# VIPL-Audio-Visual-Speech-Understanding/SBL_For_Multilingual_Lip_Reading

Measured on AMD Instinct MI355X. Metric: lip-clips/sec fwd+bwd (29x88x88), higher is better.
Workload: dtype f32 (exact 3-way bf16 split, 6 bf16 MFMA products per fp32 product, fp32 accumulate); 1 GPU; full SBL 6+6 (Conv3d stem + ResNet-18 + encoder + SBL decoder) fwd+loss+bwd (BASELINE config 3); matmul_precision=bf16x6, per_gpu_batch=32, global_batch=32, clip=29x88x88, parallelism=dp1, dropout=True, bn=train, issue=graph, hipgraph=True, decoder_streams=2, conv_weight_pack=cached (re-packed when weights change), decoder_schedule=teacher-forced runs batched, coin_patterns=8

## Files before the change

include/sbl_hip.h:

```cpp
#ifndef SBL_HIP_H
#define SBL_HIP_H
#include <stdint.h>
#ifdef __cplusplus
extern "C" {
#endif

#define SBL_ERR_INVALID (-22)
#define SBL_ABI_VERSION 1

typedef void* sbl_stream_t;

const char* sbl_last_error(void);
int sbl_abi_version(void);

int sbl_profile_begin(uint64_t* stamps, int capacity);
int sbl_profile_end(void);
int sbl_profile_used(void);
int sbl_profile_last_slot(void);
int sbl_profile_last_kernel(void);
int sbl_profile_last_route(void);

int sbl_set_matmul_precision(int terms);
int sbl_get_matmul_precision(void);
int sbl_set_tuning(int knob, int value);
// ... 52 lines not shown
int sbl_bn_bwd_apply(const float* dy, const float* y, const float* x, const float* mean, const float* invstd,
                     const float* gamma, const double* sums, float* dx, float* dres, float* dgamma, float* dbeta,
                     long rows, int C, int relu, int accumulate, sbl_stream_t stream);

int sbl_conv_weight_pack(const float* w_oihw, float* w_ohwi, float* w_dgrad , int Cout,
                         int Cin, int KH, int KW, double* zero , int nzero, sbl_stream_t stream);
int sbl_conv_wgrad_unpack(const float* dw_ohwi, float* dw_oihw, int Cout, int Cin, int KH, int KW, int accumulate,
                          sbl_stream_t stream);
int sbl_conv2d_fwd(const float* x, const float* w_ohwi, float* y, double* stats, int stats_zeroed, int NIMG, int H, int W, int Cin,
                   int Cout, int KH, int KW, int stride, int pad, void* ws, long ws_bytes, sbl_stream_t stream);
int sbl_conv2d_dgrad(const float* dy, const float* w_dgrad, float* dx, int NIMG, int H, int W, int Cin, int Cout,
                     int KH, int KW, int stride, int pad, void* ws, long ws_bytes, sbl_stream_t stream);
int sbl_conv2d_dgrad_bnstats(const float* dy, const float* w_dgrad, float* dx, int NIMG, int H, int W, int Cin, int Cout,
                             int KH, int KW, int stride, int pad, void* ws, long ws_bytes, const float* act,
                             const float* pre, const float* mean, const float* invstd, double* sums,
                             int sums_zeroed ,
                             sbl_stream_t stream);
int sbl_conv2d_dgrad_fused(const float* dy, const float* w_dgrad, float* dx, int NIMG, int H, int W, int Cin, int Cout,
                           int KH, int KW, int stride, int pad, void* ws, long ws_bytes, const float* addend,
                           const float* act, const float* pre, const float* mean, const float* invstd, const float* pre2,
                           const float* mean2, const float* invstd2, double* sums, int sums_zeroed, sbl_stream_t stream);
int sbl_conv1x1s2_dgrad_compact(const float* dy, const float* w_dgrad, float* dx_compact, int NIMG, int H, int W, int Cin,
                                int Cout, void* ws, long ws_bytes, sbl_stream_t stream);
int sbl_conv2d_wgrad(const float* x, const float* dy, float* dw_ohwi, int NIMG, int H, int W, int Cin, int Cout,
                     int KH, int KW, int stride, int pad, int dw_zeroed, sbl_stream_t stream);
int sbl_avgpool_fwd(const float* x, float* y, int NIMG, int HW, int C, sbl_stream_t stream);
int sbl_avgpool_bwd(const float* dy, float* dx, int NIMG, int HW, int C, sbl_stream_t stream);

int sbl_dropout(const float* x, float* y, long n, float p, const uint64_t* seed, uint64_t offset,
                sbl_stream_t stream);
int sbl_seed_bump(uint64_t* seed, sbl_stream_t stream);

int sbl_add_layernorm_fwd(const float* x, const float* res, const float* gamma, const float* beta, float* y,
                          float* mean, float* rstd, int M, int D, float eps, float drop_p, const uint64_t* seed,
                          uint64_t offset, sbl_stream_t stream);
int sbl_add_layernorm2_fusion_fwd(const float* x0, const float* x1, const float* res0, const float* res1, const float* gamma0,
                                  const float* gamma1, const float* beta0, const float* beta1, float* xn0, float* xn1, float* mean0,
                                  float* mean1, float* rstd0, float* rstd1, int B, const int* seg_L, int nseg, int D, float eps,
                                  float drop_p, const uint64_t* seed, uint64_t offset0, uint64_t offset1, sbl_stream_t stream);
int sbl_add_layernorm2_fwd(const float* x0, const float* x1, const float* res0, const float* res1, const float* gamma0,
                           const float* gamma1, const float* beta0, const float* beta1, float* y0, float* y1, float* mean0,
                           float* mean1, float* rstd0, float* rstd1, int M, int D, float eps, float drop_p,
                           const uint64_t* seed, uint64_t offset0, uint64_t offset1, sbl_stream_t stream);
int sbl_add_layernorm_bwd(const float* dy, const float* x, const float* res, const float* gamma, const float* mean,
                          const float* rstd, float* dz, float* dx_drop, float* dgamma, float* dbeta, int M, int D,
                          float drop_p, const uint64_t* seed, uint64_t offset, sbl_stream_t stream);
// ... 172 lines not shown
```

sbl_for_multilingual_lip_reading_amd/_lib.py:

```python
import ctypes
import os
from ctypes import c_double, c_float, c_int, c_long, c_uint64, c_void_p

_HERE = os.path.dirname(os.path.abspath(__file__))
LIB_PATH = os.path.join(_HERE, "libsbl_hip.so")

P, I, L, F, U64, D = c_void_p, c_int, c_long, c_float, c_uint64, c_double

SIGNATURES = {
    "sbl_gemm_f32": [I, I, I, I, I, P, L, P, L, P, L, P, I, P, L, I, P, P, L, P],
    "sbl_wgrad_seg_f32": [I, P, L, P, L, P, I, I, P, L, P, P],
    "sbl_wgrad_group_f32": [I, I, P, P, P, P, P, P, P, P, P, P, P, L, P],
    "sbl_colsum_f32": [P, L, P, I, I, I, P],
    "sbl_stem_conv_fwd": [P, P, P, P, I, I, I, I, P],
    "sbl_stem_bn_relu_pool_fwd": [P, P, P, P, P, P, P, I, I, I, P],
    "sbl_stem_bwd_reduce": [P, P, P, P, P, P, P, P, I, I, I, P],
    "sbl_stem_wgrad": [P, P, P, P, P, P, P, P, P, P, P, P, I, I, I, I, P],
    "sbl_stem_conv_fwd_u8": [P, P, P, P, P, P, P, P, P, I, I, I, I, I, I, I, P],
    "sbl_stem_wgrad_u8": [P, P, P, P, P, P, P, P, P, P, P, P, P, P, P, P, P, I, I, I, I, I, I, I, P],
    "sbl_bn_finalize": [P, L, P, P, F, F, P, P, I, P, P],
    "sbl_bn_eval_stats": [P, P, F, P, P, I, P],
    "sbl_bn_apply_fwd": [P, P, P, P, P, P, P, L, I, I, P],
    "sbl_bn_apply_fwd_stats": [P, P, P, L, P, P, F, F, P, P, P, P, P, P, L, I, I, P],
    "sbl_bn_bwd_reduce": [P, P, P, P, P, P, L, I, I, P, L, P],
    "sbl_bn_bwd_apply": [P, P, P, P, P, P, P, P, P, P, P, L, I, I, I, P],
    "sbl_conv_weight_pack": [P, P, P, I, I, I, I, P, I, P],
    "sbl_conv_wgrad_unpack": [P, P, I, I, I, I, I, P],
    "sbl_conv2d_fwd": [P, P, P, P, I, I, I, I, I, I, I, I, I, I, P, L, P],
    "sbl_conv2d_dgrad": [P, P, P, I, I, I, I, I, I, I, I, I, P, L, P],
    "sbl_conv2d_dgrad_bnstats": [P, P, P, I, I, I, I, I, I, I, I, I, P, L, P, P, P, P, P, I, P],
    "sbl_conv2d_dgrad_fused": [P, P, P, I, I, I, I, I, I, I, I, I, P, L, P, P, P, P, P, P, P, P, P, I, P],
    "sbl_conv1x1s2_dgrad_compact": [P, P, P, I, I, I, I, I, P, L, P],
    "sbl_conv2d_wgrad": [P, P, P, I, I, I, I, I, I, I, I, I, I, P],
    "sbl_avgpool_fwd": [P, P, I, I, I, P],
    "sbl_avgpool_bwd": [P, P, I, I, I, P],
    "sbl_dropout": [P, P, L, F, P, U64, P],
    "sbl_seed_bump": [P, P],
    "sbl_add_layernorm_fwd": [P, P, P, P, P, P, P, I, I, F, F, P, U64, P],
    "sbl_add_layernorm_bwd": [P, P, P, P, P, P, P, P, P, P, I, I, F, P, U64, P],
    "sbl_add_pe": [P, P, P, I, I, I, P],
    "sbl_rowscale": [P, P, P, L, I, P],
    "sbl_attention_fwd": [P, L, P, L, P, L, P, L, P, I, P, I, I, I, I, F, F, P, U64, P],
    "sbl_attention_bwd": [P, L, P, L, P, L, P, L, P, P, L, P, L, P, L, I, I, I, I, F, F, P, U64, P],
    "sbl_attention_seg_fwd": [P, L, P, L, P, L, P, L, P, I, P, I, I, P, I, I, F, F, P, U64, P],
    "sbl_attention_seg2_fwd": [P, P, L, P, P, L, P, P, L, P, P, L, P, P, I, I, I, P, I, I, F, F, P, U64, U64, P],
    "sbl_attention_seg_grouped_fwd": [P, L, P, L, P, L, P, L, I, I, P, I, I, I, F, F, P, U64, P],
    "sbl_gemm2_f32": [I, I, I, P, P, L, P, P, L, P, P, L, P, P, I, P, L, P],
    "sbl_gemm2_rows_f32": [I, I, I, P, P, L, P, P, L, P, P, L, P, P, I, P, L, P],
    "sbl_add_layernorm2_fwd": [P, P, P, P, P, P, P, P, P, P, P, P, P, P, I, I, F, F, P, U64, U64, P],
    "sbl_add_layernorm2_fusion_fwd": [P, P, P, P, P, P, P, P, P, P, P, P, P, P, I, P, I, I, F, F, P, U64, U64, P],
    "sbl_attention_seg_bwd": [P, L, P, L, P, L, P, L, P, P, L, P, L, P, L, I, I, P, I, I, F, F, P, U64, P],
    "sbl_embed_pe_seg_fwd": [P, L, P, P, P, I, P, I, I, I, P],
    "sbl_embed_pe_drop2_fwd": [P, P, L, P, P, P, P, I, P, I, I, I, F, P, U64, U64, P],
    "sbl_decoder_tail_fwd": [P, P, P, P, P, P, P, P, L, P, P, L, I, I, I, P, I, I, I, P],
    "sbl_embed_seg_bwd": [P, L, P, P, I, P, I, I, I, P],
# ... 84 lines not shown
```

sbl_for_multilingual_lip_reading_amd/csrc/conv.hip:

```cpp
#include "mfma_gemm.h"
#include "conv_patch.h"
#include "conv_patch_wgrad.h"

SblRouting g_sbl_route = {2, 30};
extern "C" int sbl_set_tuning(int knob, int value) {
    SBL_REQUIRE(knob == 5 || knob == 9, "sbl_set_tuning: no knob %d; the two that remain are 5 (patch-resident 3x3 / stride-1 forward / input gradient: 2 on, "
                "0 the per-tap gather kernels) and 9 (smallest map in pixels that takes the patch-resident weight gradient, 0 = never)", knob);
    if (knob == 5) {
        SBL_REQUIRE(value == 0 || value == 2, "sbl_set_tuning: knob 5 takes 2 (patch-resident kernels) or 0 (per-tap gather kernels), not %d", value);
        g_sbl_route.conv_patch = value;
    } else {
        SBL_REQUIRE(value >= 0, "sbl_set_tuning: negative value");
        g_sbl_route.conv_patch_wgrad = value;
    }
    return 0;
}

static int check_conv(const char* who, int NIMG, int H, int W, int Cin, int Cout, int KH, int KW, int stride, int pad) {
    SBL_REQUIRE(NIMG > 0 && H > 0 && W > 0, "%s: bad image dims %d %d %d", who, NIMG, H, W);
    SBL_REQUIRE(Cin % 16 == 0 && Cout % 16 == 0 && Cin >= 16 && Cout >= 16, "%s: Cin=%d Cout=%d must be multiples of 16", who, Cin, Cout);
    SBL_REQUIRE((KH == 3 && KW == 3 && pad == 1) || (KH == 1 && KW == 1 && pad == 0), "%s: only 3x3/pad1 and 1x1/pad0 (got %dx%d pad %d)", who, KH, KW, pad);
    SBL_REQUIRE(stride == 1 || stride == 2, "%s: stride %d", who, stride);
    SBL_REQUIRE(sbl_fits_u32((long)NIMG * H * W * (long)(Cin > Cout ? Cin : Cout)), "%s: tensor spans more than 2 GiB (buffer descriptor range)", who);
    SBL_REQUIRE((long)NIMG * H * W < (1L << 24) && Cin < (1 << 16) && Cout < (1 << 16), "%s: more than 2^24 pixels (24-bit index arithmetic in the gathers)", who);
// ... 112 lines not shown
    if (stats && !stats_zeroed) SBL_HIP(hipMemsetAsync(stats, 0, sizeof(double) * 2 * Cout, s));
    SBL_REQUIRE(!ws || (sbl_aligned16(ws) && ws_bytes >= (long)sizeof(int) * kConvWsCounters), "sbl_conv2d_fwd: workspace unaligned or < 16 KiB");
    if (KH == 3 && stride == 1) {
        bool done;
        const PatchEpi pe{y, stats, nullptr, nullptr, nullptr, nullptr, nullptr, nullptr, nullptr, nullptr};
        if (stats) done = sbl_launch_conv_patch<false, 1>(x, w, pe, NIMG, H, W, Cin, Cout, SBL_KID_CONV_FWD, s);
        else done = sbl_launch_conv_patch<false, 0>(x, w, pe, NIMG, H, W, Cin, Cout, SBL_KID_CONV_FWD, s);
        if (done) {
            SBL_LAUNCH_CHECK("sbl_conv2d_fwd(patch)");
            return 0;
        }
    }
    if (conv_pm_ok(Ho, Wo, KH, stride)) {
        with_fwd_epi(y, N, stats, rows_pm(NIMG, Ho * Wo), [&](const auto& e) { launch_conv_pm<false>(x, w, g, e, M, N, K, Cin, SBL_KID_CONV_FWD, s); });
        SBL_LAUNCH_CHECK("sbl_conv2d_fwd(pm)");
        return 0;
    }
    const ConvTile tile = conv_tile(N, (long)sbl_cdiv(M, 128) * sbl_cdiv(N, 128), (long)sbl_cdiv(M, 128) * sbl_cdiv(N, 64), true, false);
    with_fwd_epi(y, N, stats, kRowsDirect, [&](const auto& e) { launch_conv_gemm<false>(x, w, g, e, tile, M, N, K, SBL_KID_CONV_FWD, ws, ws_bytes, s); });
    SBL_LAUNCH_CHECK("sbl_conv2d_fwd");
    return 0;
}

struct DgradClass { ConvGeom g; int lin[4]; int M, K, ph, pw; };
static int conv2d_dgrad_impl(const float* dy, const float* wt, float* dx, int NIMG, int H, int W, int Cin, int Cout,
                             int KH, int KW, int stride, int pad, void* ws, long ws_bytes, sbl_stream_t stream,
                             const DgradFuse& f, int compact_out) {
    hipStream_t s = (hipStream_t)stream;
    if (int e = check_conv("sbl_conv2d_dgrad", NIMG, H, W, Cin, Cout, KH, KW, stride, pad)) return e;
    SBL_REQUIRE(dy && wt && dx && sbl_aligned16(dy) && sbl_aligned16(wt), "sbl_conv2d_dgrad: null/unaligned pointer");
    const int Ho = out_dim(H, KH, stride, pad), Wo = out_dim(W, KW, stride, pad);
    const bool fused = f.addend || f.sums;
    if (f.sums) {
        SBL_REQUIRE(f.y && f.x && f.mean && f.inv && (!f.x2 || (f.mean2 && f.inv2)), "sbl_conv2d_dgrad_fused: incomplete BatchNorm operands");
        if (!f.sums_zeroed) SBL_HIP(hipMemsetAsync(f.sums, 0, sizeof(double) * (f.x2 ? 4 : 2) * Cin, s));
    }
    SBL_REQUIRE(!f.addend || f.add_class00 == (stride == 2), "sbl_conv2d_dgrad_fused: the compact addend belongs to stride-2 convolutions (and only to them)");
    SBL_REQUIRE(!compact_out || (KH == 1 && stride == 2 && !fused), "sbl_conv2d_dgrad: compact output is the 1x1 / stride-2 case");
    if (stride == 2) {
        const int N = Cin;
        if (KH == 1 && !compact_out) SBL_HIP(hipMemsetAsync(dx, 0, sizeof(float) * (size_t)NIMG * H * W * Cin, s));
        DgradClass cls[4];
        int nc = 0;
        for (int ph = 0; ph < 2; ++ph)
            for (int pw = 0; pw < 2; ++pw) {
                DgradClass c{ConvGeom{NIMG, (H - ph + 1) / 2, (W - pw + 1) / 2, Ho, Wo, Cout, KH, KW, stride, pad, 1, ph, pw, 0, {0, 0, 0, 0}, {0, 0, 0, 0}}, {0, 0, 0, 0}, 0, 0, ph, pw};
                sbl_geom_finish(c.g);
                for (int kh = 0; kh < KH; ++kh)
                    for (int kw = 0; kw < KW; ++kw)
                        if (((ph + pad - kh) & 1) == 0 && ((pw + pad - kw) & 1) == 0) {
                            c.g.tkh[c.g.ntaps] = kh; c.g.tkw[c.g.ntaps] = kw; c.lin[c.g.ntaps] = kh * KW + kw;
                            ++c.g.ntaps;
                        }
                c.M = NIMG * c.g.OH * c.g.OW;
                c.K = c.g.ntaps * Cout;
                if (c.g.ntaps == 0 || c.M == 0) continue;
                int at = nc++;
                while (at > 0 && cls[at - 1].K < c.K) { cls[at] = cls[at - 1]; --at; }
                cls[at] = c;
            }
        if (nc == 0) return 0;
        SplitCtl sc{nullptr, nullptr, nullptr, sbl_next_stamp_slot(SBL_KID_CONV_DGRAD)};
        const int cmap = compact_out ? 0 : 1;
        long t128 = 0, t128x64 = 0;
        for (int i = 0; i < nc; ++i) {
            t128 += (long)sbl_cdiv(cls[i].M, 128) * sbl_cdiv(N, 128);
            t128x64 += (long)sbl_cdiv(cls[i].M, 128) * sbl_cdiv(N, 64);
        }
        const ConvTile tile = conv_tile(N, t128, t128x64, false, f.sums != nullptr);
        int t0[SBL_MAX_CLASSES + 1];
        long tt = 0;
        for (int i = 0; i <= SBL_MAX_CLASSES; ++i) {
            t0[i] = (int)tt;
            if (i < nc) tt += (long)sbl_cdiv(cls[i].M, conv_tile_m(tile)) * sbl_cdiv(N, conv_tile_n(tile));
        }
        SBL_REQUIRE(tt < (1L << 30), "sbl_conv2d_dgrad: too many tiles");
        with_dgrad_epi(dx, N, f, [&](auto make) {
            with_tile(tile, [&](auto bm, auto bn) {
                constexpr int BM = decltype(bm)::value, BN = decltype(bn)::value;
                using AL = ConvGatherKC<BM, true>;
                using BL = DenseKCTaps<BN>;
                using EPI = decltype(make(kRowsDirect, f.addend, 0L));
                ClassSet<AL, BL, EPI> cs;
                cs.nclass = nc;
                cs.tiles_n = sbl_cdiv(N, BN);
                for (int i = 0; i < SBL_MAX_CLASSES; ++i) {
                    const DgradClass& c = cls[i < nc ? i : 0];
                    const float* add = (f.addend && c.ph == 0 && c.pw == 0) ? f.addend : nullptr;
                    cs.al[i] = AL{dy, c.g, c.M};
                    cs.bl[i] = BL{wt, (long)KH * KW * Cout, N, Cout, {c.lin[0], c.lin[1], c.lin[2], c.lin[3]}};
                    cs.epi[i] = make(RowMap{cmap, c.g.OH, c.g.OW, H, W, c.ph, c.pw}, add, (long)N);
                    cs.M[i] = c.M; cs.K[i] = c.K; cs.t0[i] = t0[i];
                }
                cs.t0[SBL_MAX_CLASSES] = t0[SBL_MAX_CLASSES];
                sbl_note_route(5, sbl_route_tile(BM, BN), 0, 0);
                sbl_with_prec([&](auto p) {
                    hipLaunchKernelGGL((sbl_conv_classes_kernel<AL, BL, EPI, BM, BN, decltype(p)::value>), dim3((unsigned)tt), dim3(256), 0, s, cs, sc, N);
                });
            });
        });
        SBL_LAUNCH_CHECK("sbl_conv2d_dgrad(classes)");
        return 0;
    }
    const int M = NIMG * H * W, N = Cin, K = KH * KW * Cout;
    ConvGeom g{NIMG, H, W, Ho, Wo, Cout, KH, KW, stride, pad, 0, 0, 0, 0, {0, 0, 0, 0}, {0, 0, 0, 0}};
    sbl_geom_finish(g);
    SBL_REQUIRE(!ws || (sbl_aligned16(ws) && ws_bytes >= (long)sizeof(int) * kConvWsCounters), "sbl_conv2d_dgrad: workspace unaligned or < 16 KiB");
    if (KH == 3 && stride == 1) {
        bool done;
        const PatchEpi pe{dx, f.sums, f.addend, f.y, f.x, f.mean, f.inv, f.x2, f.mean2, f.inv2};
        if (f.sums) done = sbl_launch_conv_patch<true, 2>(dy, wt, pe, NIMG, H, W, Cout, Cin, SBL_KID_CONV_DGRAD, s);
        else if (f.addend) done = sbl_launch_conv_patch<true, 3>(dy, wt, pe, NIMG, H, W, Cout, Cin, SBL_KID_CONV_DGRAD, s);
        else done = sbl_launch_conv_patch<true, 0>(dy, wt, pe, NIMG, H, W, Cout, Cin, SBL_KID_CONV_DGRAD, s);
// ... 16 lines not shown
    SBL_LAUNCH_CHECK("sbl_conv2d_dgrad");
    return 0;
}
static const DgradFuse kNoFuse{nullptr, 0, nullptr, nullptr, nullptr, nullptr, nullptr, nullptr, nullptr, nullptr};
extern "C" int sbl_conv2d_dgrad(const float* dy, const float* wt, float* dx, int NIMG, int H, int W, int Cin, int Cout,
                                int KH, int KW, int stride, int pad, void* ws, long ws_bytes, sbl_stream_t stream) {
    return conv2d_dgrad_impl(dy, wt, dx, NIMG, H, W, Cin, Cout, KH, KW, stride, pad, ws, ws_bytes, stream, kNoFuse, 0);
}
extern "C" int sbl_conv2d_dgrad_bnstats(const float* dy, const float* wt, float* dx, int NIMG, int H, int W, int Cin, int Cout,
                                        int KH, int KW, int stride, int pad, void* ws, long ws_bytes, const float* act,
                                        const float* pre, const float* mean, const float* invstd, double* sums,
                                        int sums_zeroed, sbl_stream_t stream) {
    SBL_REQUIRE(act && pre && mean && invstd && sums, "sbl_conv2d_dgrad_bnstats: null statistics operand");
    return conv2d_dgrad_impl(dy, wt, dx, NIMG, H, W, Cin, Cout, KH, KW, stride, pad, ws, ws_bytes, stream,
                             DgradFuse{nullptr, 0, act, pre, mean, invstd, nullptr, nullptr, nullptr, sums, sums_zeroed}, 0);
}
extern "C" int sbl_conv2d_dgrad_fused(const float* dy, const float* wt, float* dx, int NIMG, int H, int W, int Cin, int Cout,
                                      int KH, int KW, int stride, int pad, void* ws, long ws_bytes, const float* addend,
                                      const float* act, const float* pre, const float* mean, const float* invstd,
                                      const float* pre2, const float* mean2, const float* invstd2, double* sums,
                                      int sums_zeroed, sbl_stream_t stream) {
    return conv2d_dgrad_impl(dy, wt, dx, NIMG, H, W, Cin, Cout, KH, KW, stride, pad, ws, ws_bytes, stream,
                             DgradFuse{addend, addend && stride == 2, act, pre, mean, invstd, pre2, mean2, invstd2, sums, sums_zeroed}, 0);
}
extern "C" int sbl_conv1x1s2_dgrad_compact(const float* dy, const float* wt, float* dx_compact, int NIMG, int H, int W, int Cin,
                                           int Cout, void* ws, long ws_bytes, sbl_stream_t stream) {
    return conv2d_dgrad_impl(dy, wt, dx_compact, NIMG, H, W, Cin, Cout, 1, 1, 2, 0, ws, ws_bytes, stream, kNoFuse, 1);
}

static inline int wgrad_splits(long target, long tiles, int K) {
    int splits = (int)((target + tiles - 1) / tiles);
    if (splits > K / 256) splits = K / 256;
    return splits < 1 ? 1 : splits;
}
extern "C" int sbl_conv2d_wgrad(const float* x, const float* dy, float* dw, int NIMG, int H, int W, int Cin, int Cout,
                                int KH, int KW, int stride, int pad, int dw_zeroed, sbl_stream_t stream) {
    hipStream_t s = (hipStream_t)stream;
    if (int e = check_conv("sbl_conv2d_wgrad", NIMG, H, W, Cin, Cout, KH, KW, stride, pad)) return e;
    SBL_REQUIRE(x && dy && dw && sbl_aligned16(x) && sbl_aligned16(dy), "sbl_conv2d_wgrad: null/unaligned pointer");
    const int Ho = out_dim(H, KH, stride, pad), Wo = out_dim(W, KW, stride, pad);
    const int M = Cout, N = KH * KW * Cin, K = NIMG * Ho * Wo;
    ConvGeom g{NIMG, Ho, Wo, H, W, Cin, KH, KW, stride, pad, 0, 0, 0, 0, {0, 0, 0, 0}, {0, 0, 0, 0}};
    sbl_geom_finish(g);
    if (!dw_zeroed) SBL_HIP(hipMemsetAsync(dw, 0, sizeof(float) * (size_t)M * N, s));
    const bool big = M >= 128 && N >= 1152 && !(stride == 2 && sbl_wg_s2_small);
    const int wg_target = stride == 2 ? sbl_wg_s2_target : (big ? 1536 : 3072);
// ... 121 lines not shown
```

sbl_for_multilingual_lip_reading_amd/csrc/tile_loaders.h:

```cpp
#pragma once
#include "sbl_common.h"

#define SBL_BK 16
#define SBL_BUF_BYTES 0x80000000u
#define SBL_OOB 0xC0000000u

typedef __amdgpu_buffer_rsrc_t sbl_rsrc;
__device__ __forceinline__ sbl_rsrc sbl_make_rsrc(const float* p) {
    return __builtin_amdgcn_make_buffer_rsrc(const_cast<float*>(p), 0, (int)SBL_BUF_BYTES, 0x00020000);
}
__device__ __forceinline__ float4 sbl_ld4(sbl_rsrc r, unsigned off) {
    const f32x4 v = __builtin_bit_cast(f32x4, __builtin_amdgcn_raw_buffer_load_b128(r, (int)off, 0, 0));
    return make_float4(v[0], v[1], v[2], v[3]);
}
__device__ __forceinline__ float sbl_ld1(sbl_rsrc r, unsigned off) {
    return __builtin_bit_cast(float, __builtin_amdgcn_raw_buffer_load_b32(r, (int)off, 0, 0));
}
static inline bool sbl_fits_u32(long elems) { return elems >= 0 && elems * 4 <= (long)SBL_BUF_BYTES; }

template <int BR, class Regs>
__device__ __forceinline__ void sbl_store_kc(float (*lds)[BR + 4], const Regs& r, int tid) {
    const int kq = (tid & 3) * 4;
#pragma unroll
    for (int ps = 0; ps < BR / 64; ++ps) {
// ... 54 lines not shown
            } else {
                r.v[ps].x = sbl_ld1(s.rs, ok && k + 0 < kend ? o + 0 : SBL_OOB);
                r.v[ps].y = sbl_ld1(s.rs, ok && k + 1 < kend ? o + 4 : SBL_OOB);
                r.v[ps].z = sbl_ld1(s.rs, ok && k + 2 < kend ? o + 8 : SBL_OOB);
                r.v[ps].w = sbl_ld1(s.rs, ok && k + 3 < kend ? o + 12 : SBL_OOB);
            }
        }
    }
    __device__ __forceinline__ void accum(const Regs&, float4&) const {}
    __device__ __forceinline__ int col(const State&) const { return 0; }
    __device__ __forceinline__ void store(float (*lds)[BR + 4], const State&, const Regs& r, int tid) const { sbl_store_kc<BR>(lds, r, tid); }
};

template <int BR>
struct DenseKCTaps {
    static constexpr bool kColSum = false;
    static constexpr bool kKC = true;
    static constexpr bool kDenseOperand = false;
    const float* p;
    long ld;
    int rows;
    int C;
    int lin[4];
    struct State {
        sbl_rsrc rs;
        unsigned ro[BR / 64];
        int kq;
    };
    struct Regs {
        float4 v[BR / 64];
    };
    __device__ __forceinline__ void init(State& s, int r0, int tid) const {
        s.rs = sbl_make_rsrc(p);
        s.kq = (tid & 3) * 4;
#pragma unroll
        for (int ps = 0; ps < BR / 64; ++ps) {
            const int r = r0 + ps * 64 + (tid >> 2);
            s.ro[ps] = r < rows ? (unsigned)(((long)r * ld + s.kq) * 4) : SBL_OOB;
        }
    }
    __device__ __forceinline__ void load(const State& s, int k0, int kend, Regs& r) const {
        const int t = k0 / C;
        int l = lin[0];
#pragma unroll
        for (int u = 1; u < 4; ++u)
            if (u == t) l = lin[u];
        const unsigned kb = (unsigned)(l * C + (k0 - t * C)) * 4;
#pragma unroll
        for (int ps = 0; ps < BR / 64; ++ps)
            r.v[ps] = sbl_ld4(s.rs, s.ro[ps] != SBL_OOB && k0 < kend ? s.ro[ps] + kb : SBL_OOB);
    }
    __device__ __forceinline__ void accum(const Regs&, float4&) const {}
    __device__ __forceinline__ int col(const State&) const { return 0; }
    __device__ __forceinline__ void store(float (*lds)[BR + 4], const State&, const Regs& r, int tid) const { sbl_store_kc<BR>(lds, r, tid); }
};

template <int BR>
struct DenseKCTapList {
    static constexpr bool kColSum = false;
    static constexpr bool kKC = true;
    static constexpr bool kDenseOperand = false;
    const float* p;
    long ld;
    int rows;
    int C;
    unsigned long long taps;
    struct State {
        sbl_rsrc rs;
        unsigned ro[BR / 64];
        int kq;
    };
    struct Regs {
        float4 v[BR / 64];
// ... 169 lines not shown
template <bool DGRAD>
__device__ __forceinline__ int conv_row_scale(const ConvGeom& g) { return DGRAD ? 1 : g.stride; }
template <bool DGRAD, bool MAYCLS = DGRAD>
__device__ __forceinline__ unsigned conv_tap_mask(const ConvGeom& g, int oh, int ow, int ntap) {
    const int sA = conv_row_scale<DGRAD>(g);
    unsigned m = 0;
    for (int t = 0; t < ntap; ++t) {
        int dh, dw;
        conv_tap_delta<DGRAD, MAYCLS>(g, t, dh, dw);
        const int ih = oh * sA + dh, iw = ow * sA + dw;
        if ((unsigned)ih < (unsigned)g.SH && (unsigned)iw < (unsigned)g.SW) m |= 1u << t;
    }
    return m;
}

template <int BR, bool DGRAD>
struct ConvGatherKC {
    static constexpr bool kColSum = false;
    static constexpr bool kKC = true;
    static constexpr bool kDenseOperand = false;
    const float* p;
    ConvGeom g;
    int rows;
    struct State {
        sbl_rsrc rs;
        int base[BR / 64];
        unsigned mask[BR / 64];
    };
    struct Regs {
        float4 v[BR / 64];
    };
    __device__ __forceinline__ void init(State& s, int r0, int tid) const {
        s.rs = sbl_make_rsrc(p);
        const int sA = conv_row_scale<DGRAD>(g);
        const int ntap = (DGRAD && g.cls) ? g.ntaps : g.KH * g.KW;
#pragma unroll
        for (int ps = 0; ps < BR / 64; ++ps) {
            const int r = r0 + ps * 64 + (tid >> 2);
            const bool ok = r < rows;
            const unsigned rr = ok ? (unsigned)r : 0u;
            const int img = (int)sbl_div(rr, g.fdHW);
            const int rem = (int)rr - img * (g.OH * g.OW);
            const int oh = (int)sbl_div((unsigned)rem, g.fdOW), ow = rem - oh * g.OW;
            s.base[ps] = (((img * g.SH + oh * sA) * g.SW + ow * sA) * g.C + (tid & 3) * 4) * 4;
            s.mask[ps] = ok ? conv_tap_mask<DGRAD>(g, oh, ow, ntap) : 0u;
        }
    }
    __device__ __forceinline__ void load(const State& s, int k0, int kend, Regs& r) const {
        const int tap = (int)sbl_div((unsigned)k0, g.fdC);
        int dh, dw;
        conv_tap_delta<DGRAD>(g, tap, dh, dw);
        const int delta = ((dh * g.SW + dw) * g.C + (k0 - tap * g.C)) * 4;
        const unsigned bit = k0 < kend ? (1u << (tap & 31)) : 0u;
#pragma unroll
        for (int ps = 0; ps < BR / 64; ++ps) r.v[ps] = sbl_ld4(s.rs, (s.mask[ps] & bit) ? (unsigned)(s.base[ps] + delta) : SBL_OOB);
    }
    __device__ __forceinline__ void accum(const Regs&, float4&) const {}
    __device__ __forceinline__ int col(const State&) const { return 0; }
    __device__ __forceinline__ void store(float (*lds)[BR + 4], const State&, const Regs& r, int tid) const { sbl_store_kc<BR>(lds, r, tid); }
};

template <int BR>
struct ConvGatherMC {
    static constexpr bool kColSum = false;
    static constexpr bool kKC = false;
    static constexpr bool kDenseOperand = false;
    const float* p;
    ConvGeom g;
    int rows;
    static constexpr int TPR = BR / 4;
    static constexpr int RPP = 256 / TPR;
    static constexpr int NP = SBL_BK / RPP;
    struct State {
        sbl_rsrc rs;
        int c, dh, dw, kr;
        bool ok;
    };
    struct Regs {
// ... 165 lines not shown
```

sbl_for_multilingual_lip_reading_amd/ops.py:

```python
import collections as _collections
import contextlib as _contextlib
import copy as _copy
import ctypes as _ct
import functools as _functools
import threading as _threading
import types as _types
import weakref as _weakref

import numpy as _np
import torch
import torch.distributed as _dist

try:
    from . import _lib
except ImportError:
    import _lib

call = _lib.call

_PRECISIONS = {"f32": 0, "bf16x6": 6, "bf16x3": 3, "bf16": 1}


def set_matmul_precision(mode):
    if mode not in _PRECISIONS:
# ... 1141 lines not shown
        call("sbl_stem_wgrad_u8" if ctx.raw else "sbl_stem_wgrad", *[_p(t) for t in src], _p(conv), _p(dpooled), _p(argmax), _p(mean),
             _p(invstd), _p(gamma), _p(beta), _p(sums), _p(dw), _p(dgamma), _p(dbeta), *dims, _s())
        return None, dw.view(64, 1, 5, 7, 7), dgamma, dbeta, None, None, None, None, None, None


def _dgrad_weight(w, w_dg):
    if w_dg is None:
        Cout, Cin, KH, KW = w.shape
        w_ohwi = torch.empty(Cout, KH, KW, Cin, device=w.device, dtype=torch.float32)
        w_dg = torch.empty(Cin, KH, KW, Cout, device=w.device, dtype=torch.float32)
        call("sbl_conv_weight_pack", _p(w.contiguous()), _p(w_ohwi), _p(w_dg), Cout, Cin, KH, KW, None, 0, _s())
    return w_dg


ConvBN = _collections.namedtuple("ConvBN", "w gamma beta running_mean running_var nbt stride momentum eps")


def _conv_geom(x, w, stride):
    NIMG, H, W, Cin = x.shape
    Cout, _, KH, KW = w.shape
    return NIMG, H, W, Cin, Cout, KH, KW, stride, (1 if KH == 3 else 0)


def conv_bn_fwd(x, c, res, relu, training, need_dg):
    g = _conv_geom(x, c.w, c.stride)
    NIMG, H, W, _, Cout, KH, KW, stride, pad = g
    Ho = (H + 2 * pad - KH) // stride + 1
    Wo = (W + 2 * pad - KW) // stride + 1
    dev = x.device
    stats, pooled_stats = _zeros_or_empty(dev, (2 * Cout,), torch.float64) if training else (None, False)
    w_ohwi, w_dg = packed_conv_weight(c.w, training and need_dg, None if pooled_stats else stats)
    conv = torch.empty(NIMG, Ho, Wo, Cout, device=dev, dtype=torch.float32)
    mean = torch.empty(Cout, device=dev, dtype=torch.float32)
    invstd = torch.empty(Cout, device=dev, dtype=torch.float32)
    y = torch.empty_like(conv)
    call("sbl_conv2d_fwd", _p(x), _p(w_ohwi), _p(conv), _p(stats), int(training), *g, _workspace().data_ptr(), WS_BYTES, _s())
    if training:
        call("sbl_bn_apply_fwd_stats", _p(conv), _p(res), _p(stats), NIMG * Ho * Wo, _p(c.running_mean), _p(c.running_var), c.momentum,
             c.eps, _p(c.gamma), _p(c.beta), _p(y), _p(mean), _p(invstd), _p(c.nbt), NIMG * Ho * Wo, Cout, int(relu), _s())
    else:
        call("sbl_bn_eval_stats", _p(c.running_mean), _p(c.running_var), c.eps, _p(mean), _p(invstd), Cout, _s())
        call("sbl_bn_apply_fwd", _p(conv), _p(res), _p(mean), _p(invstd), _p(c.gamma), _p(c.beta), _p(y), NIMG * Ho * Wo, Cout,
             int(relu), _s())
    return conv, y, mean, invstd, w_dg


def bn_bwd_reduce(dy, y, bn):
    conv, mean, invstd = bn
    Cout = conv.size(-1)
    sums = torch.empty(2 * Cout, device=conv.device, dtype=torch.float64)
    call("sbl_bn_bwd_reduce", _p(dy), _p(y), _p(conv), _p(mean), _p(invstd), _p(sums), conv.numel() // Cout, Cout, int(y is not None),
         _workspace().data_ptr(), WS_BYTES, _s())
    return sums


def bn_bwd_apply(dy, y, bn, gamma, beta, sums, with_res):
    conv, mean, invstd = bn
    Cout = conv.size(-1)
    dconv = torch.empty_like(conv)
    dres = torch.empty_like(conv) if with_res else None
    dgamma, dbeta = _gbuf(gamma), _gbuf(beta)
    acc = dgamma is not None and dbeta is not None
    if not acc:
        dgamma = torch.empty(Cout, device=conv.device, dtype=torch.float32)
        dbeta = torch.empty(Cout, device=conv.device, dtype=torch.float32)
    call("sbl_bn_bwd_apply", _p(dy), _p(y), _p(conv), _p(mean), _p(invstd), _p(gamma), _p(sums), _p(dconv), _p(dres),
         _p(dgamma), _p(dbeta), conv.numel() // Cout, Cout, int(y is not None), int(acc), _s())
    return (dconv, dres, None, None) if acc else (dconv, dres, dgamma, dbeta)


def conv_dgrad(dconv, w, w_dg, x, stride, addend=None, bn=None, bn_ds=None):
    Cin = x.size(-1)
    w_dg = _dgrad_weight(w, w_dg)
    dx = torch.empty_like(x)
    n_bn = (bn is not None) + (bn_ds is not None)
    sums, pooled = _zeros_or_empty(x.device, (2 * n_bn * Cin,), torch.float64) if n_bn else (None, False)
    head = (_p(dconv), _p(w_dg), _p(dx), *_conv_geom(x, w, stride), _workspace().data_ptr(), WS_BYTES)
    if addend is None:
        call("sbl_conv2d_dgrad_bnstats", *head, _p(x), *map(_p, bn), _p(sums), int(pooled), _s())
    else:
        call("sbl_conv2d_dgrad_fused", *head, _p(addend), _p(x if n_bn else None), *map(_p, bn or (None,) * 3), *map(_p, bn_ds or (None,) * 3),
             _p(sums), int(pooled), _s())
    return dx, sums


def conv_wgrad(x, dconv, w, stride):
    g = _conv_geom(x, w, stride)
    _, _, _, Cin, Cout, KH, KW, _, _ = g
    dev = x.device

    def launch(dw_ohwi, pooled, target, acc):
        call("sbl_conv2d_wgrad", _p(x), _p(dconv), _p(dw_ohwi), *g, int(pooled), _s())
        call("sbl_conv_wgrad_unpack", _p(dw_ohwi), _p(target), Cout, Cin, KH, KW, acc, _s())

    gw = _gbuf(w)
    if gw is None:
        dw = torch.empty_like(w)
        launch(torch.empty(Cout, KH, KW, Cin, device=dev, dtype=torch.float32), False, dw, 0)
        return dw
    side = side_stream(dev)
    side.wait_stream(torch.cuda.current_stream())
# ... 16 lines not shown
        self.act, self.bn2, self.bn_ds = y.data_ptr(), bn2, bn_ds

    def describes(self, x):
        return self.bn2 is not None and self.act == x.data_ptr()

    def deposit(self, sums, dx):
        self.sums, self.dx_ptr = sums, dx.data_ptr()

    def take(self, dy):
        if self.sums is None or self.dx_ptr != dy.data_ptr():
            return None
        sums = self.sums
        self.__init__()
        return sums


class BlockFn(torch.autograd.Function):

    @staticmethod
    def forward(ctx, x, prev, pub, c1, c2, ds, training, *params):
        _need_cuda(x, *params)
        x = x.contiguous()
        need_dx = ctx.needs_input_grad[0]
        conv1, out, mean1, invstd1, w_dg1 = conv_bn_fwd(x, c1, None, True, training, need_dx)
        res, bn_ds, saved_ds = x, None, ()
        if ds is not None:
            conv_ds, res, mean_ds, invstd_ds, w_dg_ds = conv_bn_fwd(x, ds, None, False, training, need_dx)
            bn_ds, saved_ds = (conv_ds, mean_ds, invstd_ds), (conv_ds, mean_ds, invstd_ds, w_dg_ds)
        need_dout = pub is not None and (need_dx or any(ctx.needs_input_grad[7:10]))
        conv2, y, mean2, invstd2, w_dg2 = conv_bn_fwd(out, c2, res, True, training, need_dout)
        ctx.save_for_backward(x, conv1, out, mean1, invstd1, w_dg1, conv2, y, mean2, invstd2, w_dg2, *params, *saved_ds)
        ctx.training, ctx.strides, ctx.prev, ctx.pub = training, (c1.stride, ds.stride if ds is not None else None), prev, pub
        if pub is not None:
            pub.publish(y, (conv2, mean2, invstd2), bn_ds)
        return y

    @staticmethod
    @_bw
    def backward(ctx, dy):
        if not ctx.training:
            raise _lib.SblHipError("ConvBN backward is implemented for training-mode BatchNorm only")
        x, conv1, out, mean1, invstd1, w_dg1, conv2, y, mean2, invstd2, w_dg2, *params = ctx.saved_tensors
        w1, gamma1, beta1, w2, gamma2, beta2, *ds = params
        stride1, stride_ds = ctx.strides
        need_dx = ctx.needs_input_grad[0]
        bn1, bn2 = (conv1, mean1, invstd1), (conv2, mean2, invstd2)
        dy = dy.contiguous()
        sums2 = ctx.pub.take(dy) if ctx.pub is not None else None
        sums_ds = None
        if sums2 is None:
            sums2 = bn_bwd_reduce(dy, y, bn2)
        elif ds:
            sums2, sums_ds = sums2[:sums2.numel() // 2], sums2[sums2.numel() // 2:]
        dconv2, dres, dgamma2, dbeta2 = bn_bwd_apply(dy, y, bn2, gamma2, beta2, sums2, True)
        dout, sums1 = conv_dgrad(dconv2, w2, w_dg2, out, 1, bn=bn1)
        dw2 = conv_wgrad(out, dconv2, w2, 1)
        grads_ds, addend = (), dres
        if ds:
            w_ds, gamma_ds, beta_ds, conv_ds, mean_ds, invstd_ds, w_dg_ds = ds
            bn_ds = (conv_ds, mean_ds, invstd_ds)
            if sums_ds is None:
                sums_ds = bn_bwd_reduce(dres, None, bn_ds)
            dconv_ds, _, dgamma_ds, dbeta_ds = bn_bwd_apply(dres, None, bn_ds, gamma_ds, beta_ds, sums_ds, False)
            if need_dx:
                NIMG, H, W, Cin = x.shape
                addend = torch.empty(NIMG, (H + 1) // 2, (W + 1) // 2, Cin, device=x.device, dtype=torch.float32)
                call("sbl_conv1x1s2_dgrad_compact", _p(dconv_ds), _p(_dgrad_weight(w_ds, w_dg_ds)), _p(addend), NIMG, H, W, Cin,
                     w_ds.size(0), _workspace().data_ptr(), WS_BYTES, _s())
            grads_ds = (conv_wgrad(x, dconv_ds, w_ds, stride_ds), dgamma_ds, dbeta_ds)
        dconv1, _, dgamma1, dbeta1 = bn_bwd_apply(dout, out, bn1, gamma1, beta1, sums1, False)
        dx = None
        if need_dx:
            prev = ctx.prev if ctx.prev is not None and ctx.prev.describes(x) else None
            if prev is None:
                dx, _ = conv_dgrad(dconv1, w1, w_dg1, x, stride1, addend)
            else:
                dx, sums_prev = conv_dgrad(dconv1, w1, w_dg1, x, stride1, addend, prev.bn2, prev.bn_ds)
                prev.deposit(sums_prev, dx)
        dw1 = conv_wgrad(x, dconv1, w1, stride1)
        return (dx, None, None, None, None, None, None, dw1, dgamma1, dbeta1, dw2, dgamma2, dbeta2, *grads_ds)


def basic_block(x, c1, c2, ds, training):
    pub = BlockHandoff() if training and torch.is_grad_enabled() else None
    y = BlockFn.apply(x, getattr(x, "_sbl_handoff", None), pub, c1, c2, ds, training, *c1[:3], *c2[:3], *(ds[:3] if ds is not None else ()))
    if pub is not None:
        y._sbl_handoff = pub
    return y


class AvgPoolFn(torch.autograd.Function):

    @staticmethod
    def forward(ctx, x):
        _need_cuda(x)
        x = x.contiguous()
        NIMG, H, W, C = x.shape
        y = torch.empty(NIMG, C, device=x.device, dtype=torch.float32)
        call("sbl_avgpool_fwd", _p(x), _p(y), NIMG, H * W, C, _s())
        ctx.shape = x.shape
# ... 467 lines not shown
```

Measured before the change: 1094 clips/s.

## Fuse downsample shortcut 1x1 conv with 3x3 stride-2 conv in one launch

Adds a paired forward kernel that runs the 3x3 stride-2 conv and the 1x1 stride-2 shortcut conv of a downsampling block as two tile classes in a single launch over the shared input. It also adds a paired dgrad path that appends the shortcut's gradient as an extra K-segment of the phase-(0,0) class, which removes the separate compact dgrad launch and its addend buffer. Only the forward pairing is enabled by default; the dgrad pairing sits behind a flag that is off. The goal is fewer launches and better occupancy on the small downsample layers. In exchange the dense B-loader now computes row offsets with a 24-bit multiply and carries extra branches.

```diff
diff --git a/include/sbl_hip.h b/include/sbl_hip.h
--- a/include/sbl_hip.h
+++ b/include/sbl_hip.h
@@ -98,6 +98,12 @@
                            const float* mean2, const float* invstd2, double* sums, int sums_zeroed, sbl_stream_t stream);
 int sbl_conv1x1s2_dgrad_compact(const float* dy, const float* w_dgrad, float* dx_compact, int NIMG, int H, int W, int Cin,
                                 int Cout, void* ws, long ws_bytes, sbl_stream_t stream);
+int sbl_conv2d_fwd_pair(const float* x, const float* w3_ohwi, const float* w1_ohwi, float* y3, float* y1, double* stats3,
+                        double* stats1, int stats_zeroed, int NIMG, int H, int W, int Cin, int Cout, sbl_stream_t stream);
+int sbl_conv2d_dgrad_pair(const float* dy, const float* w_dgrad, const float* dy_ds, const float* w_dgrad_ds, float* dx, int NIMG,
+                          int H, int W, int Cin, int Cout, void* ws, long ws_bytes, const float* act, const float* pre,
+                          const float* mean, const float* invstd, const float* pre2, const float* mean2, const float* invstd2,
+                          double* sums, int sums_zeroed, sbl_stream_t stream);
 int sbl_conv2d_wgrad(const float* x, const float* dy, float* dw_ohwi, int NIMG, int H, int W, int Cin, int Cout,
                      int KH, int KW, int stride, int pad, int dw_zeroed, sbl_stream_t stream);
 int sbl_avgpool_fwd(const float* x, float* y, int NIMG, int HW, int C, sbl_stream_t stream);
diff --git a/sbl_for_multilingual_lip_reading_amd/_lib.py b/sbl_for_multilingual_lip_reading_amd/_lib.py
--- a/sbl_for_multilingual_lip_reading_amd/_lib.py
+++ b/sbl_for_multilingual_lip_reading_amd/_lib.py
@@ -31,6 +31,8 @@
     "sbl_conv2d_dgrad_bnstats": [P, P, P, I, I, I, I, I, I, I, I, I, P, L, P, P, P, P, P, I, P],
     "sbl_conv2d_dgrad_fused": [P, P, P, I, I, I, I, I, I, I, I, I, P, L, P, P, P, P, P, P, P, P, P, I, P],
     "sbl_conv1x1s2_dgrad_compact": [P, P, P, I, I, I, I, I, P, L, P],
+    "sbl_conv2d_fwd_pair": [P, P, P, P, P, P, P, I, I, I, I, I, I, P],
+    "sbl_conv2d_dgrad_pair": [P, P, P, P, P, I, I, I, I, I, P, L, P, P, P, P, P, P, P, P, I, P],
     "sbl_conv2d_wgrad": [P, P, P, I, I, I, I, I, I, I, I, I, I, P],
     "sbl_avgpool_fwd": [P, P, I, I, I, P],
     "sbl_avgpool_bwd": [P, P, I, I, I, P],
diff --git a/sbl_for_multilingual_lip_reading_amd/csrc/conv.hip b/sbl_for_multilingual_lip_reading_amd/csrc/conv.hip
--- a/sbl_for_multilingual_lip_reading_amd/csrc/conv.hip
+++ b/sbl_for_multilingual_lip_reading_amd/csrc/conv.hip
@@ -158,10 +158,56 @@
     return 0;
 }
 
+extern "C" int sbl_conv2d_fwd_pair(const float* x, const float* w3, const float* w1, float* y3, float* y1, double* stats3, double* stats1,
+                                   int stats_zeroed, int NIMG, int H, int W, int Cin, int Cout, sbl_stream_t stream) {
+    hipStream_t s = (hipStream_t)stream;
+    if (int e = check_conv("sbl_conv2d_fwd_pair", NIMG, H, W, Cin, Cout, 3, 3, 2, 1)) return e;
+    SBL_REQUIRE(x && w3 && w1 && y3 && y1 && stats3 && stats1 && sbl_aligned16(x) && sbl_aligned16(w3) && sbl_aligned16(w1),
+                "sbl_conv2d_fwd_pair: null/unaligned pointer");
+    const int Ho = out_dim(H, 3, 2, 1), Wo = out_dim(W, 3, 2, 1);
+    const int M = NIMG * Ho * Wo, N = Cout;
+    ConvGeom g3{NIMG, Ho, Wo, H, W, Cin, 3, 3, 2, 1, 0, 0, 0, 0, {0, 0, 0, 0}, {0, 0, 0, 0}};
+    ConvGeom g1{NIMG, Ho, Wo, H, W, Cin, 1, 1, 2, 0, 0, 0, 0, 0, {0, 0, 0, 0}, {0, 0, 0, 0}};
+    sbl_geom_finish(g3);
+    sbl_geom_finish(g1);
+    if (!stats_zeroed) {
+        SBL_HIP(hipMemsetAsync(stats3, 0, sizeof(double) * 2 * Cout, s));
+        SBL_HIP(hipMemsetAsync(stats1, 0, sizeof(double) * 2 * Cout, s));
+    }
+    const ConvTile tile = conv_tile(N, 2L * sbl_cdiv(M, 128) * sbl_cdiv(N, 128), 2L * sbl_cdiv(M, 128) * sbl_cdiv(N, 64), true, false);
+    const long per = (long)sbl_cdiv(M, conv_tile_m(tile)) * sbl_cdiv(N, conv_tile_n(tile));
+    SBL_REQUIRE(2 * per < (1L << 30), "sbl_conv2d_fwd_pair: too many tiles");
+    SplitCtl sc{nullptr, nullptr, nullptr, sbl_next_stamp_slot(SBL_KID_CONV_FWD)};
+    with_tile(tile, [&](auto bm, auto bn) {
+        constexpr int BM = decltype(bm)::value, BN = decltype(bn)::value;
+        using AL = ConvGatherKC<BM, false>;
+        using BL = DenseKC<BN, true>;
+        using EPI = EpiStore<0, true>;
+        ClassSet<AL, BL, EPI> cs;
+        cs.nclass = 2;
+        cs.tiles_n = sbl_cdiv(N, BN);
+        for (int i = 0; i < SBL_MAX_CLASSES; ++i) {
+            const bool sh = i == 1;
+            const int K = sh ? Cin : 9 * Cin;
+            cs.al[i] = AL{x, sh ? g1 : g3, M};
+            cs.bl[i] = BL{sh ? w1 : w3, (long)K, N};
+            cs.epi[i] = epi_stats(sh ? y1 : y3, N, sh ? stats1 : stats3, kRowsDirect);
+            cs.M[i] = M; cs.K[i] = K; cs.t0[i] = (int)(i < 2 ? i * per : 2 * per);
+        }
+        cs.t0[SBL_MAX_CLASSES] = (int)(2 * per);
+        sbl_note_route(5, sbl_route_tile(BM, BN), 0, 0);
+        sbl_with_prec([&](auto p) {
+            hipLaunchKernelGGL((sbl_conv_classes_kernel<AL, BL, EPI, BM, BN, decltype(p)::value>), dim3((unsigned)(2 * per)), dim3(256), 0, s, cs, sc, N);
+        });
+    });
+    SBL_LAUNCH_CHECK("sbl_conv2d_fwd_pair");
+    return 0;
+}
+
 struct DgradClass { ConvGeom g; int lin[4]; int M, K, ph, pw; };
 static int conv2d_dgrad_impl(const float* dy, const float* wt, float* dx, int NIMG, int H, int W, int Cin, int Cout,
                              int KH, int KW, int stride, int pad, void* ws, long ws_bytes, sbl_stream_t stream,
-                             const DgradFuse& f, int compact_out) {
+                             const DgradFuse& f, int compact_out, const float* dy2 = nullptr, const float* wt2 = nullptr) {
     hipStream_t s = (hipStream_t)stream;
     if (int e = check_conv("sbl_conv2d_dgrad", NIMG, H, W, Cin, Cout, KH, KW, stride, pad)) return e;
     SBL_REQUIRE(dy && wt && dx && sbl_aligned16(dy) && sbl_aligned16(wt), "sbl_conv2d_dgrad: null/unaligned pointer");
@@ -173,6 +219,8 @@
     }
     SBL_REQUIRE(!f.addend || f.add_class00 == (stride == 2), "sbl_conv2d_dgrad_fused: the compact addend belongs to stride-2 convolutions (and only to them)");
     SBL_REQUIRE(!compact_out || (KH == 1 && stride == 2 && !fused), "sbl_conv2d_dgrad: compact output is the 1x1 / stride-2 case");
+    SBL_REQUIRE(!dy2 == !wt2 && (!dy2 || (KH == 3 && stride == 2 && pad == 1 && !f.addend && sbl_aligned16(dy2) && sbl_aligned16(wt2))),
+                "sbl_conv2d_dgrad_pair: the shortcut's gradient and weight image come together, aligned, with a 3x3 / stride-2 / pad-1 convolution and no addend");
     if (stride == 2) {
         const int N = Cin;
         if (KH == 1 && !compact_out) SBL_HIP(hipMemsetAsync(dx, 0, sizeof(float) * (size_t)NIMG * H * W * Cin, s));
@@ -189,7 +237,7 @@
                             ++c.g.ntaps;
                         }
                 c.M = NIMG * c.g.OH * c.g.OW;
-                c.K = c.g.ntaps * Cout;
+                c.K = (c.g.ntaps + (dy2 && ph == 0 && pw == 0)) * Cout;
                 if (c.g.ntaps == 0 || c.M == 0) continue;
                 int at = nc++;
                 while (at > 0 && cls[at - 1].K < c.K) { cls[at] = cls[at - 1]; --at; }
@@ -222,9 +270,10 @@
                 cs.tiles_n = sbl_cdiv(N, BN);
                 for (int i = 0; i < SBL_MAX_CLASSES; ++i) {
                     const DgradClass& c = cls[i < nc ? i : 0];
-                    const float* add = (f.addend && c.ph == 0 && c.pw == 0) ? f.addend : nullptr;
-                    cs.al[i] = AL{dy, c.g, c.M};
-                    cs.bl[i] = BL{wt, (long)KH * KW * Cout, N, Cout, {c.lin[0], c.lin[1], c.lin[2], c.lin[3]}};
+                    const bool c00 = c.ph == 0 && c.pw == 0;
+                    const float* add = (f.addend && c00) ? f.addend : nullptr;
+                    cs.al[i] = AL{dy, c.g, c.M, c00 ? dy2 : nullptr};
+                    cs.bl[i] = BL{wt, (long)KH * KW * Cout, N, Cout, {c.lin[0], c.lin[1], c.lin[2], c.lin[3]}, c00 ? wt2 : nullptr, (long)Cout, c.g.ntaps};
                     cs.epi[i] = make(RowMap{cmap, c.g.OH, c.g.OW, H, W, c.ph, c.pw}, add, (long)N);
                     cs.M[i] = c.M; cs.K[i] = c.K; cs.t0[i] = t0[i];
                 }
@@ -287,6 +336,14 @@
                                       int sums_zeroed, sbl_stream_t stream) {
     return conv2d_dgrad_impl(dy, wt, dx, NIMG, H, W, Cin, Cout, KH, KW, stride, pad, ws, ws_bytes, stream,
                              DgradFuse{addend, addend && stride == 2, act, pre, mean, invstd, pre2, mean2, invstd2, sums, sums_zeroed}, 0);
+}
+extern "C" int sbl_conv2d_dgrad_pair(const float* dy, const float* wt, const float* dy_ds, const float* wt_ds, float* dx, int NIMG, int H, int W,
+                                     int Cin, int Cout, void* ws, long ws_bytes, const float* act, const float* pre, const float* mean,
+                                     const float* invstd, const float* pre2, const float* mean2, const float* invstd2, double* sums,
+                                     int sums_zeroed, sbl_stream_t stream) {
+    SBL_REQUIRE(dy_ds && wt_ds, "sbl_conv2d_dgrad_pair: null shortcut operand");
+    return conv2d_dgrad_impl(dy, wt, dx, NIMG, H, W, Cin, Cout, 3, 3, 2, 1, ws, ws_bytes, stream,
+                             DgradFuse{nullptr, 0, act, pre, mean, invstd, pre2, mean2, invstd2, sums, sums_zeroed}, 0, dy_ds, wt_ds);
 }
 extern "C" int sbl_conv1x1s2_dgrad_compact(const float* dy, const float* wt, float* dx_compact, int NIMG, int H, int W, int Cin,
                                            int Cout, void* ws, long ws_bytes, sbl_stream_t stream) {
diff --git a/sbl_for_multilingual_lip_reading_amd/csrc/tile_loaders.h b/sbl_for_multilingual_lip_reading_amd/csrc/tile_loaders.h
--- a/sbl_for_multilingual_lip_reading_amd/csrc/tile_loaders.h
+++ b/sbl_for_multilingual_lip_reading_amd/csrc/tile_loaders.h
@@ -100,21 +100,24 @@
     int rows;
     int C;
     int lin[4];
-    struct State {
-        sbl_rsrc rs;
-        unsigned ro[BR / 64];
-        int kq;
+    const float* px;
+    long ldx;
+    int nt;
+    struct State {
+        sbl_rsrc rs;
+        int row[BR / 64];
+        unsigned kq4;
     };
     struct Regs {
         float4 v[BR / 64];
     };
     __device__ __forceinline__ void init(State& s, int r0, int tid) const {
         s.rs = sbl_make_rsrc(p);
-        s.kq = (tid & 3) * 4;
+        s.kq4 = (unsigned)(tid & 3) * 16u;
 #pragma unroll
         for (int ps = 0; ps < BR / 64; ++ps) {
             const int r = r0 + ps * 64 + (tid >> 2);
-            s.ro[ps] = r < rows ? (unsigned)(((long)r * ld + s.kq) * 4) : SBL_OOB;
+            s.row[ps] = r < rows ? r : -1;
         }
     }
     __device__ __forceinline__ void load(const State& s, int k0, int kend, Regs& r) const {
@@ -123,10 +126,18 @@
 #pragma unroll
         for (int u = 1; u < 4; ++u)
             if (u == t) l = lin[u];
-        const unsigned kb = (unsigned)(l * C + (k0 - t * C)) * 4;
+        sbl_rsrc rs = s.rs;
+        unsigned rld4 = (unsigned)ld * 4u;
+        unsigned kb4 = (unsigned)(l * C + (k0 - t * C)) * 4u;
+        if (px && t == nt) {
+            rs = sbl_make_rsrc(px);
+            rld4 = (unsigned)ldx * 4u;
+            kb4 = (unsigned)(k0 - t * C) * 4u;
+        }
+        const unsigned kv = kb4 + s.kq4;
 #pragma unroll
         for (int ps = 0; ps < BR / 64; ++ps)
-            r.v[ps] = sbl_ld4(s.rs, s.ro[ps] != SBL_OOB && k0 < kend ? s.ro[ps] + kb : SBL_OOB);
+            r.v[ps] = sbl_ld4(rs, s.row[ps] >= 0 && k0 < kend ? __umul24((unsigned)s.row[ps], rld4) + kv : SBL_OOB);
     }
     __device__ __forceinline__ void accum(const Regs&, float4&) const {}
     __device__ __forceinline__ int col(const State&) const { return 0; }
@@ -342,6 +353,7 @@
     const float* p;
     ConvGeom g;
     int rows;
+    const float* px;
     struct State {
         sbl_rsrc rs;
         int base[BR / 64];
@@ -363,17 +375,24 @@
             const int rem = (int)rr - img * (g.OH * g.OW);
             const int oh = (int)sbl_div((unsigned)rem, g.fdOW), ow = rem - oh * g.OW;
             s.base[ps] = (((img * g.SH + oh * sA) * g.SW + ow * sA) * g.C + (tid & 3) * 4) * 4;
-            s.mask[ps] = ok ? conv_tap_mask<DGRAD>(g, oh, ow, ntap) : 0u;
+            s.mask[ps] = ok ? (conv_tap_mask<DGRAD>(g, oh, ow, ntap) | (DGRAD && px ? 1u << ntap : 0u)) : 0u;
         }
     }
     __device__ __forceinline__ void load(const State& s, int k0, int kend, Regs& r) const {
         const int tap = (int)sbl_div((unsigned)k0, g.fdC);
         int dh, dw;
         conv_tap_delta<DGRAD>(g, tap, dh, dw);
+        sbl_rsrc rs = s.rs;
+        if constexpr (DGRAD) {
+            if (px && tap == g.ntaps) {
+                rs = sbl_make_rsrc(px);
+                dh = dw = 0;
+            }
+        }
         const int delta = ((dh * g.SW + dw) * g.C + (k0 - tap * g.C)) * 4;
         const unsigned bit = k0 < kend ? (1u << (tap & 31)) : 0u;
 #pragma unroll
-        for (int ps = 0; ps < BR / 64; ++ps) r.v[ps] = sbl_ld4(s.rs, (s.mask[ps] & bit) ? (unsigned)(s.base[ps] + delta) : SBL_OOB);
+        for (int ps = 0; ps < BR / 64; ++ps) r.v[ps] = sbl_ld4(rs, (s.mask[ps] & bit) ? (unsigned)(s.base[ps] + delta) : SBL_OOB);
     }
     __device__ __forceinline__ void accum(const Regs&, float4&) const {}
     __device__ __forceinline__ int col(const State&) const { return 0; }
diff --git a/sbl_for_multilingual_lip_reading_amd/ops.py b/sbl_for_multilingual_lip_reading_amd/ops.py
--- a/sbl_for_multilingual_lip_reading_amd/ops.py
+++ b/sbl_for_multilingual_lip_reading_amd/ops.py
@@ -1187,7 +1187,17 @@
     return NIMG, H, W, Cin, Cout, KH, KW, stride, (1 if KH == 3 else 0)
 
 
-def conv_bn_fwd(x, c, res, relu, training, need_dg):
+SHORTCUT_PAIR = 1
+SHORTCUT_PAIR_DGRAD = 0
+
+
+def shortcut_pairs(c1, ds, training):
+    ok = training and ds is not None and c1.stride == 2 and ds.stride == 2 \
+        and tuple(c1.w.shape[2:]) == (3, 3) and tuple(ds.w.shape[2:]) == (1, 1) and c1.w.size(0) == ds.w.size(0)
+    return bool(ok and SHORTCUT_PAIR), bool(ok and SHORTCUT_PAIR_DGRAD)
+
+
+def _conv_fwd_operands(x, c, training, need_dg):
     g = _conv_geom(x, c.w, c.stride)
     NIMG, H, W, _, Cout, KH, KW, stride, pad = g
     Ho = (H + 2 * pad - KH) // stride + 1
@@ -1196,10 +1206,28 @@
     stats, pooled_stats = _zeros_or_empty(dev, (2 * Cout,), torch.float64) if training else (None, False)
     w_ohwi, w_dg = packed_conv_weight(c.w, training and need_dg, None if pooled_stats else stats)
     conv = torch.empty(NIMG, Ho, Wo, Cout, device=dev, dtype=torch.float32)
+    return g, conv, stats, w_ohwi, w_dg
+
+
+def conv_fwd(x, c, training, need_dg):
+    g, conv, stats, w_ohwi, w_dg = _conv_fwd_operands(x, c, training, need_dg)
+    call("sbl_conv2d_fwd", _p(x), _p(w_ohwi), _p(conv), _p(stats), int(training), *g, _workspace().data_ptr(), WS_BYTES, _s())
+    return conv, stats, w_dg
+
+
+def conv_fwd_pair(x, c1, ds, need_dg):
+    g, conv1, stats1, w1, w_dg1 = _conv_fwd_operands(x, c1, True, need_dg)
+    _, conv_ds, stats_ds, w_ds, w_dg_ds = _conv_fwd_operands(x, ds, True, need_dg)
+    call("sbl_conv2d_fwd_pair", _p(x), _p(w1), _p(w_ds), _p(conv1), _p(conv_ds), _p(stats1), _p(stats_ds), 1, *g[:5], _s())
+    return (conv1, stats1, w_dg1), (conv_ds, stats_ds, w_dg_ds)
+
+
+def bn_apply_fwd(conv, stats, c, res, relu, training):
+    NIMG, Ho, Wo, Cout = conv.shape
+    dev = conv.device
     mean = torch.empty(Cout, device=dev, dtype=torch.float32)
     invstd = torch.empty(Cout, device=dev, dtype=torch.float32)
     y = torch.empty_like(conv)
-    call("sbl_conv2d_fwd", _p(x), _p(w_ohwi), _p(conv), _p(stats), int(training), *g, _workspace().data_ptr(), WS_BYTES, _s())
     if training:
         call("sbl_bn_apply_fwd_stats", _p(conv), _p(res), _p(stats), NIMG * Ho * Wo, _p(c.running_mean), _p(c.running_var), c.momentum,
              c.eps, _p(c.gamma), _p(c.beta), _p(y), _p(mean), _p(invstd), _p(c.nbt), NIMG * Ho * Wo, Cout, int(relu), _s())
@@ -1207,6 +1235,12 @@
         call("sbl_bn_eval_stats", _p(c.running_mean), _p(c.running_var), c.eps, _p(mean), _p(invstd), Cout, _s())
         call("sbl_bn_apply_fwd", _p(conv), _p(res), _p(mean), _p(invstd), _p(c.gamma), _p(c.beta), _p(y), NIMG * Ho * Wo, Cout,
              int(relu), _s())
+    return y, mean, invstd
+
+
+def conv_bn_fwd(x, c, res, relu, training, need_dg):
+    conv, stats, w_dg = conv_fwd(x, c, training, need_dg)
+    y, mean, invstd = bn_apply_fwd(conv, stats, c, res, relu, training)
     return conv, y, mean, invstd, w_dg
 
 
@@ -1234,14 +1268,19 @@
     return (dconv, dres, None, None) if acc else (dconv, dres, dgamma, dbeta)
 
 
-def conv_dgrad(dconv, w, w_dg, x, stride, addend=None, bn=None, bn_ds=None):
+def conv_dgrad(dconv, w, w_dg, x, stride, addend=None, bn=None, bn_ds=None, shortcut=None):
     Cin = x.size(-1)
     w_dg = _dgrad_weight(w, w_dg)
     dx = torch.empty_like(x)
     n_bn = (bn is not None) + (bn_ds is not None)
     sums, pooled = _zeros_or_empty(x.device, (2 * n_bn * Cin,), torch.float64) if n_bn else (None, False)
     head = (_p(dconv), _p(w_dg), _p(dx), *_conv_geom(x, w, stride), _workspace().data_ptr(), WS_BYTES)
-    if addend is None:
+    if shortcut is not None:
+        dconv_ds, w_ds, w_dg_ds = shortcut
+        call("sbl_conv2d_dgrad_pair", _p(dconv), _p(w_dg), _p(dconv_ds), _p(_dgrad_weight(w_ds, w_dg_ds)), _p(dx), *_conv_geom(x, w, stride)[:5],
+             _workspace().data_ptr(), WS_BYTES, _p(x if n_bn else None), *map(_p, bn or (None,) * 3), *map(_p, bn_ds or (None,) * 3),
+             _p(sums), int(pooled), _s())
+    elif addend is None:
         call("sbl_conv2d_dgrad_bnstats", *head, _p(x), *map(_p, bn), _p(sums), int(pooled), _s())
     else:
         call("sbl_conv2d_dgrad_fused", *head, _p(addend), _p(x if n_bn else None), *map(_p, bn or (None,) * 3), *map(_p, bn_ds or (None,) * 3),
@@ -1304,15 +1343,24 @@
         _need_cuda(x, *params)
         x = x.contiguous()
         need_dx = ctx.needs_input_grad[0]
-        conv1, out, mean1, invstd1, w_dg1 = conv_bn_fwd(x, c1, None, True, training, need_dx)
+        pair, pair_dgrad = shortcut_pairs(c1, ds, training)
+        if pair:
+            (conv1, stats1, w_dg1), (conv_ds, stats_ds, w_dg_ds) = conv_fwd_pair(x, c1, ds, need_dx)
+            out, mean1, invstd1 = bn_apply_fwd(conv1, stats1, c1, None, True, training)
+        else:
+            conv1, out, mean1, invstd1, w_dg1 = conv_bn_fwd(x, c1, None, True, training, need_dx)
         res, bn_ds, saved_ds = x, None, ()
         if ds is not None:
-            conv_ds, res, mean_ds, invstd_ds, w_dg_ds = conv_bn_fwd(x, ds, None, False, training, need_dx)
+            if pair:
+                res, mean_ds, invstd_ds = bn_apply_fwd(conv_ds, stats_ds, ds, None, False, training)
+            else:
+                conv_ds, res, mean_ds, invstd_ds, w_dg_ds = conv_bn_fwd(x, ds, None, False, training, need_dx)
             bn_ds, saved_ds = (conv_ds, mean_ds, invstd_ds), (conv_ds, mean_ds, invstd_ds, w_dg_ds)
         need_dout = pub is not None and (need_dx or any(ctx.needs_input_grad[7:10]))
         conv2, y, mean2, invstd2, w_dg2 = conv_bn_fwd(out, c2, res, True, training, need_dout)
         ctx.save_for_backward(x, conv1, out, mean1, invstd1, w_dg1, conv2, y, mean2, invstd2, w_dg2, *params, *saved_ds)
         ctx.training, ctx.strides, ctx.prev, ctx.pub = training, (c1.stride, ds.stride if ds is not None else None), prev, pub
+        ctx.pair_dgrad = pair_dgrad
         if pub is not None:
             pub.publish(y, (conv2, mean2, invstd2), bn_ds)
         return y
@@ -1337,14 +1385,16 @@
         dconv2, dres, dgamma2, dbeta2 = bn_bwd_apply(dy, y, bn2, gamma2, beta2, sums2, True)
         dout, sums1 = conv_dgrad(dconv2, w2, w_dg2, out, 1, bn=bn1)
         dw2 = conv_wgrad(out, dconv2, w2, 1)
-        grads_ds, addend = (), dres
+        grads_ds, addend, shortcut = (), dres, None
         if ds:
             w_ds, gamma_ds, beta_ds, conv_ds, mean_ds, invstd_ds, w_dg_ds = ds
             bn_ds = (conv_ds, mean_ds, invstd_ds)
             if sums_ds is None:
                 sums_ds = bn_bwd_reduce(dres, None, bn_ds)
             dconv_ds, _, dgamma_ds, dbeta_ds = bn_bwd_apply(dres, None, bn_ds, gamma_ds, beta_ds, sums_ds, False)
-            if need_dx:
+            if need_dx and ctx.pair_dgrad:
+                addend, shortcut = None, (dconv_ds, w_ds, w_dg_ds)
+            elif need_dx:
                 NIMG, H, W, Cin = x.shape
                 addend = torch.empty(NIMG, (H + 1) // 2, (W + 1) // 2, Cin, device=x.device, dtype=torch.float32)
                 call("sbl_conv1x1s2_dgrad_compact", _p(dconv_ds), _p(_dgrad_weight(w_ds, w_dg_ds)), _p(addend), NIMG, H, W, Cin,
@@ -1355,9 +1405,9 @@
         if need_dx:
             prev = ctx.prev if ctx.prev is not None and ctx.prev.describes(x) else None
             if prev is None:
-                dx, _ = conv_dgrad(dconv1, w1, w_dg1, x, stride1, addend)
+                dx, _ = conv_dgrad(dconv1, w1, w_dg1, x, stride1, addend, shortcut=shortcut)
             else:
-                dx, sums_prev = conv_dgrad(dconv1, w1, w_dg1, x, stride1, addend, prev.bn2, prev.bn_ds)
+                dx, sums_prev = conv_dgrad(dconv1, w1, w_dg1, x, stride1, addend, prev.bn2, prev.bn_ds, shortcut)
                 prev.deposit(sums_prev, dx)
         dw1 = conv_wgrad(x, dconv1, w1, stride1)
         return (dx, None, None, None, None, None, None, dw1, dgamma1, dbeta1, dw2, dgamma2, dbeta2, *grads_ds)
```

Measured after the change: 1098 clips/s, median of 6. No clear change (+0.3%).
